# arthurmensch/modl

Hardware: AMD Instinct MI355X
Metric: samples/sec through DictFact.partial_fit at k=256, p=10k (higher is better)
Workload: dtype f32

## Files before the change

### include/modl_hip.h

```cpp
#ifndef MODL_HIP_H
#define MODL_HIP_H

#include <stddef.h>
#include <stdint.h>

#ifdef __cplusplus
extern "C" {
#endif

#define MODL_ABI_VERSION 5

#define MODL_MAX_COMPONENTS 4096

#define MODL_OK 0
#define MODL_EINVAL (-1)
#define MODL_ENOMEM (-2)
#define MODL_ESTATE (-3)
#define MODL_ENOGPU (-4)
#define MODL_ENORCCL (-5)
#define MODL_ERCCL (-6)
#define MODL_ETIMEOUT (-7)

#define MODL_F32 0
#define MODL_F64 1

#define MODL_AGG_MASKED 0
#define MODL_AGG_FULL 1
#define MODL_AGG_AVERAGE 2

#define MODL_OPT_VARIATIONAL 0
#define MODL_OPT_SGD 1

#define MODL_FLAG_NO_RIDER 1
#define MODL_FLAG_GEMM_STAMPS 2

int modl_abi_version(void);
int modl_max_components(void);
int modl_device_count(void);
const char *modl_error_string(int code);
#define MODL_DEBUG_CD_SPARSE_PCT 1
#define MODL_DEBUG_CD_SPLIT 2
#define MODL_DEBUG_CD_STAMPS 3
#define MODL_DEBUG_BCD_ACC 5
#define MODL_DEBUG_ATOM_STAMPS 6
#define MODL_DEBUG_BCD_TINY 7
#define MODL_DEBUG_STAGE_AHEAD 8
#define MODL_DEBUG_BCD_PERSIST 9
#define MODL_DEBUG_STATS_RESIDENT 10
#define MODL_DEBUG_RECSYS_FUSED 11
#define MODL_DEBUG_ATOM_MWG 12
#define MODL_DEBUG_BCD_FEW 13
#define MODL_DEBUG_ATOM_PIPE 14
int modl_debug_set(int what, int64_t value);
int modl_is_diag_build(void);

typedef struct modl_rk modl_rk;
int modl_rk_create(uint64_t seed, modl_rk **out);
void modl_rk_destroy(modl_rk *rk);
int modl_rk_seed(modl_rk *rk, uint64_t seed);
int modl_rk_random(modl_rk *rk, uint32_t *out);
int modl_rk_randint(modl_rk *rk, uint64_t high, int64_t *out);
int modl_rk_double(modl_rk *rk, double *out);
int modl_rk_binomial(modl_rk *rk, int64_t n, double p, int64_t *out);
int modl_rk_permutation(modl_rk *rk, int64_t n, int64_t *h_out);
int modl_rk_get_mt_state(const modl_rk *rk, uint32_t *h_key624, int32_t *pos);
int modl_rk_set_mt_state(modl_rk *rk, const uint32_t *h_key624, int32_t pos);
int modl_rk_shuffle_i64(modl_rk *rk, int64_t *h_x, int64_t n);
int modl_rk_shuffle_trace(modl_rk *rk, int64_t n, int64_t *h_trace, int64_t *h_swaps);
int modl_apply_swaps_rows(void *h_base, int64_t n, size_t row_bytes, const int64_t *h_swaps);
int modl_apply_swaps_rows_device(void *d_base, int64_t n, size_t row_bytes, const int64_t *h_swaps,
                                 void *stream);

typedef struct modl_sampler modl_sampler;
int modl_sampler_create(int64_t range, int rand_size, int replacement, uint64_t seed, modl_sampler **out);
void modl_sampler_destroy(modl_sampler *s);
int modl_sampler_yield_subset(modl_sampler *s, double reduction, int64_t *h_out, int64_t *n_out);
int modl_sampler_get(modl_sampler *s, int64_t *range, int64_t *lim_inf, int64_t *lim_sup, int64_t *h_box);
size_t modl_sampler_state_bytes(const modl_sampler *s);
int modl_sampler_get_state(const modl_sampler *s, void *h_buf, size_t bytes);
int modl_sampler_set_state(modl_sampler *s, const void *h_buf, size_t bytes);

int modl_batch_weight(int64_t count, int64_t batch_size, double learning_rate, double offset, double *out);


size_t modl_enet_regression_workspace(int dtype, int64_t b, int64_t k, int multi_gram);
int modl_enet_regression_single_gram_f32(const float *d_G, float *d_Dx, const float *d_X, int64_t ldx,
                                         int64_t p, float *d_code, const int64_t *d_indices, int64_t b,
                                         int64_t k, float l1_ratio, float alpha, int positive, float tol,
                                         int max_iter, int32_t *d_sweeps, void *d_ws, size_t ws_bytes,
                                         void *stream);
int modl_enet_regression_single_gram_f64(const double *d_G, double *d_Dx, const double *d_X, int64_t ldx,
                                         int64_t p, double *d_code, const int64_t *d_indices, int64_t b,
                                         int64_t k, double l1_ratio, double alpha, int positive, double tol,
                                         int max_iter, int32_t *d_sweeps, void *d_ws, size_t ws_bytes,
                                         void *stream);
int modl_enet_regression_multi_gram_f32(const float *d_G, float *d_Dx, const float *d_X, int64_t ldx,
                                        int64_t p, float *d_code, const int64_t *d_indices, int64_t b,
                                        int64_t k, float l1_ratio, float alpha, int positive, float tol,
                                        int max_iter, int32_t *d_sweeps, void *d_ws, size_t ws_bytes,
                                        void *stream);
int modl_enet_regression_multi_gram_f64(const double *d_G, double *d_Dx, const double *d_X, int64_t ldx,
                                        int64_t p, double *d_code, const int64_t *d_indices, int64_t b,
                                        int64_t k, double l1_ratio, double alpha, int positive, double tol,
                                        int max_iter, int32_t *d_sweeps, void *d_ws, size_t ws_bytes,
                                        void *stream);
int modl_update_G_average_f32(float *d_G_average, const float *d_G, const float *d_w_sample, int64_t b,
                              int64_t k, void *stream);
int modl_update_G_average_f64(double *d_G_average, const double *d_G, const double *d_w_sample, int64_t b,
                              int64_t k, void *stream);

int modl_enet_norm_f32(const float *d_v, int64_t rows, int64_t n, int64_t ld, int64_t inc, float l1_ratio,
                       float *d_out_norm, void *stream);
int modl_enet_norm_f64(const double *d_v, int64_t rows, int64_t n, int64_t ld, int64_t inc, double l1_ratio,
                       double *d_out_norm, void *stream);
int modl_enet_projection_f32(const float *d_v, float *d_out, int64_t rows, int64_t n, int64_t ld, int64_t inc,
                             const float *d_radius, float l1_ratio, void *stream);
int modl_enet_projection_f64(const double *d_v, double *d_out, int64_t rows, int64_t n, int64_t ld,
// ... 202 lines not shown
```

### modl_amd/_lib.py

```python
import ctypes as C
import os

_HERE = os.path.dirname(os.path.abspath(__file__))
LIB_PATH = os.path.join(_HERE, 'libmodl_hip.so')

MODL_F32, MODL_F64 = 0, 1
FLAG_NO_RIDER, FLAG_GEMM_STAMPS = 1, 2
DEBUG_CD_SPARSE_PCT = 1
DEBUG_CD_SPLIT = 2
DEBUG_BCD_ACC = 5
DEBUG_ATOM_STAMPS = 6
DEBUG_BCD_TINY = 7
DEBUG_STAGE_AHEAD = 8
DEBUG_BCD_PERSIST = 9
DEBUG_STATS_RESIDENT = 10
DEBUG_RECSYS_FUSED = 11
DEBUG_ATOM_MWG = 12
DEBUG_BCD_FEW = 13
DEBUG_ATOM_PIPE = 14
AGG = {'masked': 0, 'full': 1, 'average': 2}
OPT = {'variational': 0, 'sgd': 1}


class ModlError(RuntimeError):
    pass


class SomfDesc(C.Structure):
    _fields_ = [('dtype', C.c_int32), ('k', C.c_int32), ('p', C.c_int64), ('n_samples', C.c_int64),
                ('G_agg', C.c_int32), ('Dx_agg', C.c_int32), ('optimizer', C.c_int32), ('code_pos', C.c_int32),
                ('comp_pos', C.c_int32), ('max_iter', C.c_int32), ('code_alpha', C.c_double),
                ('code_l1_ratio', C.c_double), ('comp_l1_ratio', C.c_double), ('tol', C.c_double),
                ('step_size', C.c_double), ('max_batch', C.c_int32), ('flags', C.c_int32)]


class SomfState(C.Structure):
    _fields_ = [('d_Dt', C.c_void_p), ('d_Bt', C.c_void_p), ('d_C', C.c_void_p), ('d_code', C.c_void_p),
                ('d_comp_norm', C.c_void_p), ('d_G', C.c_void_p), ('d_Dx_average', C.c_void_p),
                ('d_G_average', C.c_void_p)]


class SomfBatch(C.Structure):
    _fields_ = [('d_X', C.c_void_p), ('ldx', C.c_int64), ('b', C.c_int32), ('s', C.c_int32),
                ('h_sample_idx', C.c_void_p), ('h_subset', C.c_void_p), ('h_order', C.c_void_p),
                ('h_w_sample', C.c_void_p), ('w', C.c_double), ('reduction', C.c_double),
                ('b_global', C.c_int64)]


class ProfEntry(C.Structure):
    _fields_ = [('name', C.c_char_p), ('ms_total', C.c_double), ('launches', C.c_int64), ('calls', C.c_int64)]


def _load():
    if os.environ.get('MODL_AMD_DIAG') == '1':
        path = os.path.join(_HERE, 'libmodl_hip_diag.so')
        if not os.path.exists(path):
            raise ImportError('modl_amd: MODL_AMD_DIAG=1 but %s is missing (make -C modl_amd/csrc)' % path)
        return C.CDLL(path)
    override = os.environ.get('MODL_HIP_LIBRARY')
    if override:
        if not os.path.exists(override):
            raise ImportError('modl_amd: MODL_HIP_LIBRARY=%s does not exist' % override)
        return C.CDLL(os.path.abspath(override))
    if not os.path.exists(LIB_PATH):
        raise ImportError(
            'modl_amd: %s is missing. Build it with `python -c "import __graft_entry__ as g; g.build()"` '
            'or `make -C modl_amd/csrc` (needs hipcc, --offload-arch=gfx950). There is no CPU fallback.' % LIB_PATH)
    try:
        return C.CDLL(LIB_PATH)
    except OSError as e:
        raise ImportError('modl_amd: cannot load %s: %s' % (LIB_PATH, e))


_vp, _i32, _i64, _u64, _f64, _sz = C.c_void_p, C.c_int32, C.c_int64, C.c_uint64, C.c_double, C.c_size_t
_P = C.POINTER


def bind(lib):
    def _sig(name, restype, *argtypes):
        f = getattr(lib, name)
        f.restype = restype
        f.argtypes = list(argtypes)
        return f

    _sig('modl_abi_version', C.c_int)
    _sig('modl_max_components', C.c_int)
    _sig('modl_device_count', C.c_int)
    _sig('modl_error_string', C.c_char_p, C.c_int)
    _sig('modl_debug_set', C.c_int, C.c_int, _i64)
    _sig('modl_is_diag_build', C.c_int)
# ... 121 lines not shown
```

### modl_amd/csrc/somf_step.hip

```cpp
#include <algorithm>
#include <atomic>
#include <chrono>
#include <condition_variable>
#include <mutex>
#include <thread>
#include <cstdlib>
#include <cstring>
#include <dlfcn.h>
#include <sched.h>
#include <new>
#include <vector>

#include "gemm_dense.hpp"
#include "gemm_wide.hpp"
#include "gemm_resident.hpp"
#include "kernels.hpp"

namespace modl {
std::atomic<int> g_stats_resident{1};

enum Section { SEC_CODE_GEMM = 0, SEC_CODE_SOLVE, SEC_STATS_GEMM, SEC_STATS_APPLY, SEC_DICT, SEC_COUNT };
static const char *kSectionNames[SEC_COUNT] = {"code_gemm", "code_solve", "stats_gemm", "stats_apply", "dict_update"};

constexpr int kStageSlots = 8;
constexpr int kProfPool = 2048;
#ifndef MODL_STAT_BM
#define MODL_STAT_BM 64
#define MODL_STAT_BN 64
#endif
#ifndef MODL_STAT_BK
#define MODL_STAT_BK 0
#endif
constexpr int kStatBM = MODL_STAT_BM, kStatBN = MODL_STAT_BN, kStatBK = MODL_STAT_BK;

template <typename T> struct EpiDxAverage {
    T *Dx; T *avg; const int64_t *idx; const T *w_sample; int64_t k; T alpha;
    __device__ __forceinline__ void operator()(int64_t i, int64_t j, T v) const {
        T *a = avg + (idx ? idx[i] : i) * k + j;
        const T ws = w_sample[i];
        T cur = *a * ((T)1 - ws);
        cur = cur + (alpha * v) * ws;
        *a = cur;
        Dx[i * k + j] = cur;
    }
};

template <typename T> __device__ __forceinline__ bool stats_pow2(T b) {
    if constexpr (sizeof(T) == 4) return (__float_as_uint(b) & 0x007fffffu) == 0 && b > (T)0 && b < (T)1e30;
    else return (__double_as_longlong(b) & 0x000fffffffffffffll) == 0 && b > (T)0 && b < (T)1e300;
}
template <typename T> __device__ __forceinline__ T stats_value(T v, T old, T beta, T wt, T bdiv, int replace, bool p2, T rinv) {
    const T x = replace ? v : wt * v;
    const T q = p2 ? x * rinv : x / bdiv;
    return replace ? q : old * beta + q;
}
template <typename T> struct EpiStats {
    static constexpr bool rmw = true;
    typedef T vec4 __attribute__((ext_vector_type(4)));
    T *out; int64_t ld; T beta, wt, bdiv; int replace; T *mirror;
    __device__ __forceinline__ T load(int64_t m, int64_t n) const { return out[m * ld + n]; }
    __device__ __forceinline__ void store(int64_t m, int64_t n, T v, T old) const {
        const bool p2 = stats_pow2(bdiv);
        const T nv = stats_value(v, old, beta, wt, bdiv, replace, p2, (T)1 / bdiv);
        out[m * ld + n] = nv;
        if (mirror) mirror[m * ld + n] = nv;
    }
    __device__ __forceinline__ void operator()(int64_t m, int64_t n, T v) const { store(m, n, v, load(m, n)); }
    bool vec4_ok() const {
        return ld % 4 == 0 && reinterpret_cast<uintptr_t>(out) % (4 * sizeof(T)) == 0 &&
               reinterpret_cast<uintptr_t>(mirror) % (4 * sizeof(T)) == 0;
    }
    __device__ __forceinline__ vec4 load4(int64_t m, int64_t n) const { return *reinterpret_cast<const vec4 *>(out + m * ld + n); }
    __device__ __forceinline__ void store4(int64_t m, int64_t n, vec4 v, vec4 old) const {
        const bool p2 = stats_pow2(bdiv);
        const T rinv = (T)1 / bdiv;
        vec4 nv;
#pragma unroll
        for (int c = 0; c < 4; ++c) nv[c] = stats_value(v[c], old[c], beta, wt, bdiv, replace, p2, rinv);
        *reinterpret_cast<vec4 *>(out + m * ld + n) = nv;
        if (mirror) *reinterpret_cast<vec4 *>(mirror + m * ld + n) = nv;
    }
};

template <typename T> struct EpiStatsRows {
    static constexpr bool rmw = true;
    T *out; int64_t ld; const int32_t *rows; T beta, wt, bdiv; int replace; T *mirror;
    __device__ __forceinline__ T load(int64_t m, int64_t n) const { return out[(int64_t)rows[m] * ld + n]; }
    __device__ __forceinline__ void store(int64_t m, int64_t n, T v, T old) const {
        const T nv = stats_value(v, old, beta, wt, bdiv, replace, stats_pow2(bdiv), (T)1 / bdiv);
        out[(int64_t)rows[m] * ld + n] = nv;
        if (mirror) mirror[m * ld + n] = nv;
    }
    __device__ __forceinline__ void operator()(int64_t m, int64_t n, T v) const { store(m, n, v, load(m, n)); }
};

template <typename T> struct PrepArgs {
// ... 366 lines not shown
int solve_codes(modl_somf_plan *pl, hipStream_t st, const T *G, int64_t g_stride, const int64_t *g_idx, T *Dx,
                const T *xnorm2, T *code, const int64_t *d_idx, int b, int32_t *d_sweeps, int *nl, T *H0buf, T *Fbuf,
                T *scatter_dst = nullptr, const int64_t *scatter_idx = nullptr, const int64_t *h_gidx = nullptr) {
    const modl_somf_desc &d = pl->d;
    const int k = d.k;
    if (d.code_l1_ratio == 0.0 && chol_blocked(k, sizeof(T), g_stride == 0)) {
        if (g_stride && g_idx && !h_gidx) return MODL_EINVAL;
        T *Linv = reinterpret_cast<T *>(pl->dws + pl->off_Linv);
        MODL_TRY(ridge_solve_wide<T>(st, G, g_stride, h_gidx, Fbuf, Linv, Dx, b, k, (T)d.code_alpha, code, d_idx));
        *nl += 2;
        if (scatter_dst) {
            hipLaunchKernelGGL((scatter_rows_T_kernel<T, int64_t>), dim3((unsigned)b), dim3(256), 0, st, scatter_dst,
                               (int64_t)k, scatter_idx, (int64_t)b, (int64_t)k, Dx, (int64_t)k);
            MODL_LAUNCH_CHECK();
            ++*nl;
        }
        return MODL_OK;
    }
    if (d.code_l1_ratio == 0.0) {
        const int nmat = g_stride ? b : 1;
        if (ridge_small_applies<T>(k)) {
            MODL_TRY(launch_ridge_small<T>(st, G, g_stride, g_idx, Dx, b, k, (T)d.code_alpha, code, d_idx));
            *nl += 1;
        } else {
            MODL_TRY(launch_cholesky<T>(st, G, g_stride, g_idx, Fbuf, k, (T)d.code_alpha, nmat));
            MODL_TRY(launch_chol_solve<T>(st, Fbuf, g_stride ? (int64_t)k * k : 0, Dx, b, k, code, d_idx));
            *nl += 2;
        }
        if (scatter_dst) {
            hipLaunchKernelGGL((scatter_rows_T_kernel<T, int64_t>), dim3((unsigned)b), dim3(256), 0, st, scatter_dst,
                               (int64_t)k, scatter_idx, (int64_t)b, (int64_t)k, code, (int64_t)k);
            MODL_LAUNCH_CHECK();
            ++*nl;
        }
        return MODL_OK;
    }
    const T *H0 = nullptr;
    (void)H0buf;
    CdArgs<T> a;
    a.G = G; a.g_stride = g_stride; a.g_idx = g_idx; a.Dx = Dx; a.xnorm2 = xnorm2; a.H0 = H0; a.code = code;
    a.idx = d_idx;
    a.code2 = scatter_dst; a.idx2 = scatter_idx;
    a.g_pad_rows = (G == reinterpret_cast<const T *>(pl->dws + pl->off_G)) ? 16 : 0;
    if (!g_stride && pl->ld_gpad && k <= 1024) {
        T *Gp = reinterpret_cast<T *>(pl->dws + pl->off_Gpad);
        MODL_TRY(launch_cd_pad_gram<T>(st, G, k, Gp, pl->ld_gpad));
        ++*nl;
        a.G = Gp; a.ldg = pl->ld_gpad; a.g_pad_rows = 16;
    }
    a.sweeps = d_sweeps; a.b = b; a.k = k;
    a.alpha = (T)((T)d.code_alpha * (T)d.code_l1_ratio);
    a.beta = (T)((double)(T)d.code_alpha * (1.0 - (double)(T)d.code_l1_ratio));
    a.tol = (T)d.tol; a.max_iter = d.max_iter; a.positive = d.code_pos;
    if (k > 1024) {
        a.G = G; a.ldg = 0; a.g_pad_rows = 0;
        if (!g_stride) {
            Operand A, B;
            A.ptr = code; A.si = k; A.sk = 1; A.gi = gather64(d_idx);
            B.ptr = G; B.si = k; B.sk = 1;
            EpiStore<T> epi{H0buf, k, (T)1};
            SplitWs none;
            MODL_TRY((launch_gemm<T, EpiStore<T>>(st, A, B, b, k, k, epi, none, nl, 512, 1)));
            a.H0 = H0buf;
        }
        MODL_TRY(launch_cd_wide<T>(st, a));
        ++*nl;
        return MODL_OK;
    }
    if (g_stride && k >= 32 && (cd_split_enabled() || !cd_one_wave_covers(k)) && !cd_split_applies<T>(a)) {
        if (!pl->Gslots) {
            pl->Gslots_bytes = cd_per_sample_scratch_bytes(sizeof(T), d.max_batch, k);
            MODL_HIP(hipMalloc(&pl->Gslots, pl->Gslots_bytes));
            MODL_HIP(hipMemsetAsync(pl->Gslots, 0, pl->Gslots_bytes, st));
        }
        MODL_TRY(launch_cd_per_sample<T>(st, a, static_cast<T *>(pl->Gslots), pl->Gslots_bytes));
        *nl += 2;
        return MODL_OK;
    }
    MODL_TRY(launch_cd<T>(st, a));
    ++*nl;
    return MODL_OK;
}

constexpr int64_t kResidentMinRows = 4096;

template <typename T, class Epi0, class Epi1>
int stats_pair(hipStream_t st, const DenseOperand &A0, const DenseOperand &B0, int64_t M0, int64_t N0, const Epi0 &e0,
               const DenseOperand &A1, const DenseOperand &B1, int64_t M1, int64_t N1, const Epi1 &e1, int64_t K,
               const SplitWs &sws, int *launches, unsigned long long *dbg = nullptr) {
    if constexpr (std::is_same<T, float>::value) {
        auto P0 = plan_stats<Epi0>(A0, B0, M0, N0, K, e0);
        if (P0.ok && M1 >= kResidentMinRows && N1 <= 256 && K % 4 == 0 && !dbg && g_stats_resident.load(std::memory_order_relaxed)) {
            auto W = plan_wide<16, Epi1>(A1, B1, M1, N1, K, e1);
            if (W.ok) {
                static const int ncu = [] {
                    int dev = 0;
                    hipDeviceProp_t prop;
                    if (hipGetDevice(&dev) == hipSuccess && hipGetDeviceProperties(&prop, dev) == hipSuccess)
                        return prop.multiProcessorCount;
                    return 256;
                }();
                return launch_gemm_stats_resident_pair<16, Epi0, Epi1>(st, P0, W, ncu, launches);
            }
        }
        if (P0.ok && cdiv(M1, 64) >= 1024 && !dbg) {
            auto W = plan_wide<32, Epi1>(A1, B1, M1, N1, K, e1);
            if (W.ok) return launch_gemm_stats_wide_pair<32, Epi0, Epi1, 256, 8, 0, true>(st, P0, W, launches);
        }
        auto P1 = plan_stats<Epi1>(A1, B1, M1, N1, K, e1);
        if (P0.ok && P1.ok) {
            P1.dbg = dbg;
            return launch_gemm_stats_pair<Epi0, Epi1>(st, P0, P1, launches);
        }
    }
    DenseProblem<T, Epi0> P0;
    P0.epi = e0;
    bool ok0 = true;
    if (M0 > 0) {
        P0 = plan_dense<T, Epi0>(A0, B0, M0, N0, K, e0, nullptr, 0);
        ok0 = P0.ok;
    }
    auto P1 = plan_dense<T, Epi1>(A1, B1, M1, N1, K, e1, nullptr, 0, 512, 1, kStatBM, kStatBN);
    if (ok0 && P1.ok)
        return launch_gemm_dense_pair<T, true, true, Epi0, true, true, Epi1, kStatBM, kStatBN, kStatBK>(st, P0, P1, launches);
    if (M0 > 0) MODL_TRY((launch_gemm_dense<T, Epi0>(st, A0, B0, M0, N0, K, e0, sws, launches)));
    return launch_gemm_dense<T, Epi1>(st, A1, B1, M1, N1, K, e1, sws, launches);
}

template <typename T>
int phase1(modl_somf_plan *pl, const modl_somf_state *stt, const modl_somf_batch *bt, T *delta, hipStream_t st,
           bool two_phase) {
    const modl_somf_desc &d = pl->d;
    const int k = d.k, b = bt->b;
    const int64_t p = d.p, s = bt->s;
    if (!stt || !stt->d_Dt || !stt->d_code || (two_phase && !delta)) return MODL_EINVAL;
    if (!stt->d_Bt || !stt->d_C || bt->b_global <= 0) return MODL_EINVAL;
    if (d.G_agg == MODL_AGG_FULL && !stt->d_G) return MODL_EINVAL;
    if (d.G_agg == MODL_AGG_AVERAGE && !stt->d_G_average) return MODL_EINVAL;
    if (d.Dx_agg == MODL_AGG_AVERAGE && !stt->d_Dx_average) return MODL_EINVAL;
    MODL_TRY(stage_batch<T>(pl, bt, st));
    ++pl->prof_step;
    char *P = pl->dws + pl->off_params;
    const int64_t *d_idx = pl->has_idx ? reinterpret_cast<const int64_t *>(P + pl->po_idx) : nullptr;
    const int32_t *d_subset = pl->has_subset ? reinterpret_cast<const int32_t *>(P + pl->po_subset) : nullptr;
    const T *d_wsample = reinterpret_cast<const T *>(P + pl->po_wsample);
    const T *X = static_cast<const T *>(bt->d_X);
    const T *Dt = static_cast<const T *>(stt->d_Dt);
    T *code = static_cast<T *>(stt->d_code);
    T *xnorm = reinterpret_cast<T *>(pl->dws + pl->off_xnorm);
    T *Dx = reinterpret_cast<T *>(pl->dws + pl->off_Dx);
    T *H0 = reinterpret_cast<T *>(pl->dws + pl->off_H0);
    T *Gbuf = reinterpret_cast<T *>(pl->dws + pl->off_G);
    T *Fbuf = reinterpret_cast<T *>(pl->dws + pl->off_F);
    SplitWs sws{pl->dws + pl->off_split, pl->split_bytes};
    int32_t *d_sweeps = reinterpret_cast<int32_t *>(pl->dws + pl->off_sweeps);
    if (pl->hist) d_sweeps = pl->hist + (pl->hist_n++ % pl->hist_cap) * (int64_t)d.max_batch;
    pl->last_sweeps_ptr = d_sweeps;
    pl->last_b = b;
    const T red = (T)bt->reduction;

    T *Dsb = reinterpret_cast<T *>(pl->dws + pl->off_Ds);
    T *Xsb = reinterpret_cast<T *>(pl->dws + pl->off_Xs);
    T *codeb = reinterpret_cast<T *>(pl->dws + pl->off_codeb);
    const int64_t s_pad = (s + 3) / 4 * 4;
    const bool cd_on_compact = d.code_l1_ratio != 0.0 && d.G_agg != MODL_AGG_AVERAGE;
    T *cb = codeb;
    if (!d_idx) cb = code;

    T *ws_split = reinterpret_cast<T *>(sws.ptr);
    const size_t ws_elems = sws.bytes / sizeof(T);
    bool ride = false;
    pl->ride_pending = false;
    pl->head_pending = false;
    {
        ProfScope ps(pl, st, SEC_CODE_GEMM);
        const T *Dsrc = Dt, *Xsrc = X;
        int64_t ldxs = bt->ldx;
        const bool need_sub = d_subset && (d.Dx_agg != MODL_AGG_FULL || d.G_agg != MODL_AGG_FULL);
        PrepArgs<T> pa;
        pa.X = X; pa.ldx = bt->ldx; pa.p = p; pa.b = b; pa.xnorm = xnorm; pa.n_norm = (d.code_l1_ratio != 0.0) ? b : 0;
        pa.Dt = Dt; pa.subset = d_subset; pa.s = s; pa.k = k; pa.Ds = Dsb; pa.n_rows = need_sub ? (int)cdiv(s, kPrepRows) : 0;
        pa.s_pad = s_pad; pa.Xs = Xsb; pa.gx = (int)std::min<int64_t>(cdiv(s_pad, 256), 64);
        pa.n_cols = (need_sub && d.Dx_agg != MODL_AGG_FULL) ? pa.gx * b : 0;
        const size_t row_bytes = sizeof(T) * (size_t)p;
        pa.fuse_cols = (pa.n_cols > 0 && pa.n_norm == b && row_bytes <= 64 * 1024 &&
                        reinterpret_cast<uintptr_t>(X) % 16 == 0 && (bt->ldx * sizeof(T)) % 16 == 0) ? 1 : 0;
        if (pa.fuse_cols) pa.n_cols = 0;
        pa.code = code; pa.idx = d_idx; pa.codeb = codeb; pa.n_code = (cd_on_compact && d_idx) ? (int)cdiv(b, kPrepRows) : 0;
        const bool proper = need_sub && s > 0 && s < p;
        ride = proper && d.Dx_agg != MODL_AGG_FULL && !(d.flags & MODL_FLAG_NO_RIDER) && cdiv(p, 64) < 1024;
        if (ride) pl->step_id = (pl->step_id == 0x7fffffff) ? 1 : pl->step_id + 1;
        pa.stamp = ride ? reinterpret_cast<int32_t *>(pl->dws + pl->off_stamp) : nullptr;
        pa.pos = reinterpret_cast<int32_t *>(pl->dws + pl->off_pos);
        pa.step = pl->step_id;
        if (need_sub) {
            Dsrc = Dsb;
            if (d.Dx_agg != MODL_AGG_FULL) { Xsrc = Xsb; ldxs = s_pad; }
        }
        const int n_prep = pa.n_norm + pa.n_rows + pa.n_cols + pa.n_code;
        if (n_prep > 0) {
            hipLaunchKernelGGL((prep_kernel<T>), dim3((unsigned)n_prep), dim3(256), pa.fuse_cols ? row_bytes : 0, st, pa);
            MODL_LAUNCH_CHECK();
            ++ps.launches;
        }
        DenseOperand A, B;
        int64_t Kdim;
        T scale;
        if (d.Dx_agg == MODL_AGG_FULL) {
            A.ptr = X; A.si = bt->ldx; A.sk = 1;
            B.ptr = Dt; B.si = 1; B.sk = k;
            Kdim = p; scale = 1;
        } else {
            A.ptr = Xsrc; A.si = ldxs; A.sk = 1;
            B.ptr = Dsrc; B.si = 1; B.sk = k;
            Kdim = s; scale = red;
        }
        DenseOperand Dg;
        Dg.ptr = Dsrc; Dg.si = 1; Dg.sk = k;
        const bool want_G = d.G_agg != MODL_AGG_FULL;
        bool paired = false;
        if (want_G && A.si != 1) {
            EpiStore<T> epiG{Gbuf, k, red};
            const size_t half = ws_elems / 2;
            constexpr int kPairTarget = 256;
            auto PG = plan_dense<T, EpiStore<T>>(Dg, Dg, k, k, s, epiG, ws_split + half, ws_elems - half, kPairTarget, 64, 64, 64, true);
            if (d.Dx_agg == MODL_AGG_AVERAGE) {
                EpiDxAverage<T> epi{Dx, static_cast<T *>(stt->d_Dx_average), d_idx, d_wsample, k, scale};
                auto PD = plan_dense<T, EpiDxAverage<T>>(A, B, b, k, Kdim, epi, ws_split, half, kPairTarget);
                if (PD.ok && PG.ok) {
                    MODL_TRY((launch_gemm_dense_pair<T, false, true, EpiDxAverage<T>, true, true, EpiStore<T>>(st, PD, PG,
                                                                                                                &ps.launches)));
                    paired = true;
                }
            } else {
                EpiStore<T> epi{Dx, k, scale};
                auto PD = plan_dense<T, EpiStore<T>>(A, B, b, k, Kdim, epi, ws_split, half, kPairTarget);
                if (PD.ok && PG.ok) {
                    MODL_TRY((launch_gemm_dense_pair<T, false, true, EpiStore<T>, true, true, EpiStore<T>>(st, PD, PG,
                                                                                                            &ps.launches)));
                    paired = true;
                }
            }
        }
        if (!paired) {
            if (d.Dx_agg == MODL_AGG_AVERAGE) {
                EpiDxAverage<T> epi{Dx, static_cast<T *>(stt->d_Dx_average), d_idx, d_wsample, k, scale};
                MODL_TRY((launch_gemm_dense<T, EpiDxAverage<T>>(st, A, B, b, k, Kdim, epi, sws, &ps.launches)));
            } else {
                EpiStore<T> epi{Dx, k, scale};
                MODL_TRY((launch_gemm_dense<T, EpiStore<T>>(st, A, B, b, k, Kdim, epi, sws, &ps.launches)));
            }
            if (want_G) {
                EpiStore<T> epi{Gbuf, k, red};
                MODL_TRY((launch_gemm_dense<T, EpiStore<T>>(st, Dg, Dg, k, k, s, epi, sws, &ps.launches)));
            }
        }
        if (d.G_agg == MODL_AGG_AVERAGE) {
            MODL_TRY(launch_update_G_average<T>(st, static_cast<T *>(stt->d_G_average), d_idx, Gbuf, d_wsample, b, k));
            ++ps.launches;
        }
    }
    {
        ProfScope ps(pl, st, SEC_CODE_SOLVE);
        if (d.G_agg == MODL_AGG_AVERAGE) {
            const T *Gavg = static_cast<const T *>(stt->d_G_average);
            MODL_TRY(solve_codes<T>(pl, st, Gavg, (int64_t)k * k, d_idx, Dx, xnorm, code, d_idx, b, d_sweeps,
                                    &ps.launches, H0, Fbuf, nullptr, nullptr, bt->h_sample_idx));
        } else {
            const T *G = (d.G_agg == MODL_AGG_FULL) ? static_cast<const T *>(stt->d_G) : Gbuf;
            if (cd_on_compact) {
                MODL_TRY(solve_codes<T>(pl, st, G, 0, nullptr, Dx, xnorm, cb, nullptr, b, d_sweeps, &ps.launches, H0, Fbuf,
                                        d_idx ? code : nullptr, d_idx));
            } else {
                MODL_TRY(solve_codes<T>(pl, st, G, 0, nullptr, Dx, xnorm, code, d_idx, b, d_sweeps, &ps.launches, H0, Fbuf));
            }
        }
    }
    {
        ProfScope ps(pl, st, SEC_STATS_GEMM);
        if (!cd_on_compact && d_idx) {
            hipLaunchKernelGGL((gather_rows_T_kernel<T, int64_t>), dim3((unsigned)b), dim3(256), 0, st, code, (int64_t)k,
                               d_idx, (int64_t)b, (int64_t)b, (int64_t)k, codeb, (int64_t)k);
            MODL_LAUNCH_CHECK();
            ++ps.launches;
        }
        DenseOperand Cd;
        Cd.ptr = cb; Cd.si = 1; Cd.sk = k;
        DenseOperand Xo;
        Xo.ptr = X; Xo.si = 1; Xo.sk = bt->ldx;
        DenseOperand Xso;
        Xso.ptr = Xsb; Xso.si = 1; Xso.sk = s_pad;
        const int replace = d.optimizer == MODL_OPT_SGD;
        const T beta = (T)(1.0 - bt->w), wt = (T)bt->w, bdiv = (T)bt->b_global;
        T *Bt = static_cast<T *>(stt->d_Bt);
        T *mC = two_phase ? delta : nullptr, *mB = two_phase ? delta + (size_t)k * k : nullptr;
        EpiStats<T> eC{static_cast<T *>(stt->d_C), k, beta, wt, bdiv, replace, mC};
        if (ride) {
            EpiStatsRows<T> eBs{Bt, k, d_subset, beta, wt, bdiv, replace, mB};
            const bool gstamps = (d.flags & MODL_FLAG_GEMM_STAMPS) != 0;
            MODL_TRY((stats_pair<T>(st, Cd, Cd, k, k, eC, Xso, Cd, s, k, eBs, b, sws, &ps.launches,
                                    gstamps ? reinterpret_cast<unsigned long long *>(pl->dws + pl->off_gstamps) : nullptr)));
            StatsRider &R = pl->rider;
            R.X = X; R.ldx = bt->ldx; R.code = cb; R.b = b; R.p = p; R.Bt = stt->d_Bt;
            R.stamp = reinterpret_cast<const int32_t *>(pl->dws + pl->off_stamp); R.step = pl->step_id;
            R.beta = (double)beta; R.wt = (double)wt; R.bdiv = (double)bdiv; R.replace = replace; R.consumed = 0;
            pl->ride_pending = true;
        } else {
            EpiStats<T> eB{Bt, k, beta, wt, bdiv, replace, d_subset ? nullptr : mB};
            MODL_TRY((stats_pair<T>(st, Cd, Cd, k, k, eC, Xo, Cd, p, k, eB, b, sws, &ps.launches)));
            if (two_phase && d_subset && s > 0) {
                hipLaunchKernelGGL((gather_rows_T_kernel<T, int32_t>), dim3((unsigned)s), dim3(256), 0, st, Bt, (int64_t)k,
                                   d_subset, s, s, (int64_t)k, mB, (int64_t)k);
                MODL_LAUNCH_CHECK();
                ++ps.launches;
            }
        }
        if (two_phase) {
            pl->head_pending = true;
            pl->head_elems = (int64_t)k * k + (d_subset ? s : p) * (int64_t)k;
        }
    }
    return MODL_OK;
// ... 850 lines not shown
```

Baseline: 1.161 million.

## Add register-resident split-K MFMA kernel for paired code/Gram products

Adds a specialized kernel for the paired Dx = X·D and G = DᵀD products in the code step. Each block owns a 32x32 tile, loads its K-slice directly from global memory into registers with no LDS staging, splits K across up to 8 waves, and reduces the partial sums through shared memory. The Gram product computes only upper-triangular tiles and mirrors them. The new path is the default when the eligibility checks pass, and a new flag restores the generic paired dense GEMM. The trade-off is heavier register use and a ceiling on K per split, in return for lower tile overhead and roughly half the Gram work.

```diff
diff --git a/include/modl_hip.h b/include/modl_hip.h
--- a/include/modl_hip.h
+++ b/include/modl_hip.h
@@ -33,6 +33,7 @@
 
 #define MODL_FLAG_NO_RIDER 1
 #define MODL_FLAG_GEMM_STAMPS 2
+#define MODL_FLAG_SPLIT_PRODUCTS 4
 
 int modl_abi_version(void);
 int modl_max_components(void);
diff --git a/modl_amd/_lib.py b/modl_amd/_lib.py
--- a/modl_amd/_lib.py
+++ b/modl_amd/_lib.py
@@ -5,7 +5,7 @@
 LIB_PATH = os.path.join(_HERE, 'libmodl_hip.so')
 
 MODL_F32, MODL_F64 = 0, 1
-FLAG_NO_RIDER, FLAG_GEMM_STAMPS = 1, 2
+FLAG_NO_RIDER, FLAG_GEMM_STAMPS, FLAG_SPLIT_PRODUCTS = 1, 2, 4
 DEBUG_CD_SPARSE_PCT = 1
 DEBUG_CD_SPLIT = 2
 DEBUG_BCD_ACC = 5
diff --git a/modl_amd/csrc/gemm_code.hpp b/modl_amd/csrc/gemm_code.hpp
--- /dev/null
+++ b/modl_amd/csrc/gemm_code.hpp
@@ -0,0 +1,220 @@
+#pragma once
+#include "gemm_dense.hpp"
+
+namespace modl {
+
+constexpr int kCodeTile = 32;
+constexpr int kCodeWaves = 8;
+constexpr int kCodeBK = 32;
+constexpr int kCodeNKT = 5;
+constexpr int kCodeMaxKps = 192;
+
+template <class Epi> struct CodeProblem {
+    DenseOperand A, B;
+    int64_t M = 0, N = 0, K = 0, kps = 0;
+    Epi epi;
+    int tn = 0, tm = 0, splits = 1, sym = 0;
+    __host__ __device__ int tiles() const { return sym ? tm * (tm + 1) / 2 : tn * tm; }
+};
+
+template <class Epi>
+CodeProblem<Epi> code_problem(const DenseProblem<float, Epi> &P, bool sym) {
+    CodeProblem<Epi> C;
+    C.A = P.A; C.B = P.B; C.M = P.M; C.N = P.N; C.K = P.K; C.kps = P.kps; C.epi = P.epi;
+    C.tm = (int)cdiv(P.M, kCodeTile); C.tn = (int)cdiv(P.N, kCodeTile);
+    C.splits = P.splits; C.sym = sym ? 1 : 0;
+    return C;
+}
+
+template <class Epi>
+bool code_eligible(const DenseProblem<float, Epi> &P, bool a_along_k) {
+    if (!P.ok || P.A.unal || P.B.unal) return false;
+    if (a_along_k ? P.A.sk != 1 : P.A.si != 1) return false;
+    if (P.B.si != 1) return false;
+    if (P.splits < 1 || P.splits > kCodeWaves) return false;
+    if (P.kps % kCodeBK != 0 || P.kps > kCodeMaxKps) return false;
+    if ((int64_t)kCodeTile * P.A.si + (kCodeMaxKps + 1) * P.A.sk >= ((int64_t)1 << 30)) return false;
+    if ((int64_t)kCodeTile * P.B.si + (kCodeMaxKps + 1) * P.B.sk >= ((int64_t)1 << 30)) return false;
+    return true;
+}
+
+__device__ __forceinline__ void code_swap32(float &a, float &b) {
+    auto r = __builtin_amdgcn_permlane32_swap(__float_as_uint(a), __float_as_uint(b), false, false);
+    a = __uint_as_float(r[0]);
+    b = __uint_as_float(r[1]);
+}
+
+template <bool FULL, int NKT>
+__device__ __forceinline__ void code_load_rows(float (&f)[NKT * (kCodeBK / 2)], const float *base, unsigned sk, unsigned ic,
+                                               int krem, int nkt, int lane) {
+    const unsigned h = lane >> 5;
+#pragma unroll
+    for (int t = 0; t < NKT; ++t)
+        if (t < nkt) {
+#pragma unroll
+            for (int u = 0; u < kCodeBK / 2; ++u) {
+                const int j = t * (kCodeBK / 2) + u;
+                unsigned kl = 2 * j + h;
+                if (!FULL) kl = ((int)kl < krem) ? kl : (unsigned)(krem - 1);
+                f[j] = *reinterpret_cast<const float *>(reinterpret_cast<const char *>(base) + (ic + kl * sk) * 4u);
+            }
+        }
+}
+template <int NKT>
+__device__ __forceinline__ void code_fix_rows(float (&f)[NKT * (kCodeBK / 2)], int krem, int nkt, int lane) {
+    const int h = lane >> 5;
+#pragma unroll
+    for (int t = 0; t < NKT; ++t)
+        if (t < nkt) {
+#pragma unroll
+            for (int u = 0; u < kCodeBK / 2; ++u) {
+                const int j = t * (kCodeBK / 2) + u;
+                f[j] = (2 * j + h < krem) ? f[j] : 0.f;
+            }
+        }
+}
+
+template <bool FULL, int NKT>
+__device__ __forceinline__ void code_load_k(float (&f)[NKT * (kCodeBK / 2)], const float *base, unsigned row, int krem,
+                                            int nkt, int lane) {
+    const unsigned h = lane >> 5;
+#pragma unroll
+    for (int t = 0; t < NKT; ++t)
+        if (t < nkt) {
+#pragma unroll
+            for (int q = 0; q < 4; ++q) {
+                unsigned kl = kCodeBK * t + 8 * q + 4 * h;
+                if (!FULL) kl = ((int)kl < krem) ? kl : 0u;
+                const float4 v = *reinterpret_cast<const float4 *>(reinterpret_cast<const char *>(base) + (row + kl) * 4u);
+                float *d = &f[t * (kCodeBK / 2) + 4 * q];
+                d[0] = v.x; d[1] = v.y; d[2] = v.z; d[3] = v.w;
+            }
+        }
+}
+template <bool FULL, int NKT>
+__device__ __forceinline__ void code_fix_k(float (&f)[NKT * (kCodeBK / 2)], int krem, int nkt, int lane) {
+    const int h = lane >> 5;
+#pragma unroll
+    for (int t = 0; t < NKT; ++t)
+        if (t < nkt) {
+#pragma unroll
+            for (int q = 0; q < 4; ++q) {
+                float *d = &f[t * (kCodeBK / 2) + 4 * q];
+                if (!FULL) {
+                    const int kl = kCodeBK * t + 8 * q + 4 * h;
+#pragma unroll
+                    for (int c = 0; c < 4; ++c) d[c] = (kl + c < krem) ? d[c] : 0.f;
+                }
+                code_swap32(d[0], d[1]);
+                code_swap32(d[2], d[3]);
+                const float x = d[1];
+                d[1] = d[2];
+                d[2] = x;
+            }
+        }
+}
+
+template <class Epi, bool AK, int NKT>
+__device__ __forceinline__ void gemm_code_pass(const CodeProblem<Epi> &P, int64_t m0, int64_t n0, int64_t k_begin, int64_t k_end,
+                                               int lane, Mma<float>::acc_t &acc, Mma<float>::acc_t &acc2) {
+    using MT = Mma<float>;
+    const int krem = (int)(k_end - k_begin), nkt = (krem + kCodeBK - 1) / kCodeBK;
+    const int i = lane & 31;
+    const unsigned ia = (unsigned)((m0 + i < P.M) ? i : P.M - 1 - m0), ib = (unsigned)((n0 + i < P.N) ? i : P.N - 1 - n0);
+    const float *pa = static_cast<const float *>(P.A.ptr) + m0 * P.A.si + k_begin * P.A.sk;
+    const float *pb = static_cast<const float *>(P.B.ptr) + n0 + k_begin * P.B.sk;
+    const unsigned ska = (unsigned)P.A.sk, skb = (unsigned)P.B.sk, rowa = ia * (unsigned)P.A.si;
+    float a[NKT * (kCodeBK / 2)], b[NKT * (kCodeBK / 2)];
+    if (krem == nkt * kCodeBK) {
+        if (AK) code_load_k<true, NKT>(a, pa, rowa, krem, nkt, lane);
+        else code_load_rows<true, NKT>(a, pa, ska, ia, krem, nkt, lane);
+        code_load_rows<true, NKT>(b, pb, skb, ib, krem, nkt, lane);
+        if (AK) code_fix_k<true, NKT>(a, krem, nkt, lane);
+    } else {
+        if (AK) code_load_k<false, NKT>(a, pa, rowa, krem, nkt, lane);
+        else code_load_rows<false, NKT>(a, pa, ska, ia, krem, nkt, lane);
+        code_load_rows<false, NKT>(b, pb, skb, ib, krem, nkt, lane);
+        if (AK) code_fix_k<false, NKT>(a, krem, nkt, lane);
+        else code_fix_rows<NKT>(a, krem, nkt, lane);
+        code_fix_rows<NKT>(b, krem, nkt, lane);
+    }
+#pragma unroll
+    for (int t = 0; t < NKT; ++t)
+        if (t < nkt) {
+#pragma unroll
+            for (int u = 0; u < kCodeBK / 2; ++u) {
+                const int j = t * (kCodeBK / 2) + u;
+                if (u & 1) acc2 = MT::mma(a[j], b[j], acc2);
+                else acc = MT::mma(a[j], b[j], acc);
+            }
+        }
+}
+
+template <class Epi, bool AK>
+__device__ __forceinline__ void gemm_code_tile(const CodeProblem<Epi> &P, int bx, int by, float (*part)[16][64]) {
+    using MT = Mma<float>;
+    const int lane = threadIdx.x & 63, w = __builtin_amdgcn_readfirstlane((int)(threadIdx.x >> 6));
+    const int64_t m0 = (int64_t)by * kCodeTile, n0 = (int64_t)bx * kCodeTile;
+    if (w < P.splits) {
+        const int64_t k_begin = (int64_t)w * P.kps, k_end = (k_begin + P.kps < P.K) ? k_begin + P.kps : P.K;
+        MT::acc_t acc, acc2;
+#pragma unroll
+        for (int r = 0; r < MT::NACC; ++r) { acc[r] = 0; acc2[r] = 0; }
+        constexpr int64_t kPass = kCodeNKT * kCodeBK;
+        gemm_code_pass<Epi, AK, kCodeNKT>(P, m0, n0, k_begin, k_begin + kPass < k_end ? k_begin + kPass : k_end, lane, acc, acc2);
+        if (k_begin + kPass < k_end)
+            gemm_code_pass<Epi, AK, (kCodeMaxKps - kCodeNKT * kCodeBK) / kCodeBK>(P, m0, n0, k_begin + kPass, k_end, lane, acc, acc2);
+#pragma unroll
+        for (int r = 0; r < MT::NACC; ++r) part[w][r][lane] = acc[r] + acc2[r];
+    }
+    __syncthreads();
+    const bool mirror = P.sym && bx > by;
+    const int splits = P.splits;
+    for (int e = (int)threadIdx.x; e < MT::NACC * 64; e += (int)blockDim.x) {
+        const int r = e >> 6, l = e & 63;
+        float x[kCodeWaves];
+#pragma unroll
+        for (int z = 0; z < kCodeWaves; ++z) x[z] = part[z < splits ? z : splits - 1][r][l];
+        float v = x[0];
+        if (splits > 1) {
+            v = 0.f;
+#pragma unroll
+            for (int z = 0; z < kCodeWaves; ++z) v += (z < splits) ? x[z] : 0.f;
+        }
+        const int64_t m = m0 + MT::acc_row(l, r), n = n0 + MT::acc_col(l, r);
+        if (m < P.M && n < P.N) {
+            P.epi(m, n, v);
+            if (mirror) P.epi(n, m, v);
+        }
+    }
+}
+
+template <class Epi0, class Epi1>
+__global__ __launch_bounds__(kCodeWaves * 64) void gemm_code_pair_kernel(CodeProblem<Epi0> P0, CodeProblem<Epi1> P1) {
+    __shared__ float part[kCodeWaves][16][64];
+    int id = (int)blockIdx.x;
+    const int t0 = P0.tiles();
+    if (id < t0) {
+        gemm_code_tile<Epi0, true>(P0, id % P0.tn, id / P0.tn, part);
+    } else {
+        id -= t0;
+        int r = 0;
+        while (id >= P1.tn - r) { id -= P1.tn - r; ++r; }
+        gemm_code_tile<Epi1, false>(P1, r + id, r, part);
+    }
+}
+
+template <class Epi0, class Epi1>
+int launch_gemm_code_pair(hipStream_t stream, const DenseProblem<float, Epi0> &P0, const DenseProblem<float, Epi1> &P1,
+                          int *launches = nullptr) {
+    const CodeProblem<Epi0> C0 = code_problem(P0, false);
+    const CodeProblem<Epi1> C1 = code_problem(P1, true);
+    const int waves = C0.splits > C1.splits ? C0.splits : C1.splits;
+    hipLaunchKernelGGL((gemm_code_pair_kernel<Epi0, Epi1>), dim3((unsigned)(C0.tiles() + C1.tiles())), dim3(64 * waves), 0,
+                       stream, C0, C1);
+    MODL_LAUNCH_CHECK();
+    if (launches) ++*launches;
+    return MODL_OK;
+}
+
+}
diff --git a/modl_amd/csrc/somf_step.hip b/modl_amd/csrc/somf_step.hip
--- a/modl_amd/csrc/somf_step.hip
+++ b/modl_amd/csrc/somf_step.hip
@@ -12,6 +12,7 @@
 #include <vector>
 
 #include "gemm_dense.hpp"
+#include "gemm_code.hpp"
 #include "gemm_wide.hpp"
 #include "gemm_resident.hpp"
 #include "kernels.hpp"
@@ -544,6 +545,19 @@
     return MODL_OK;
 }
 
+template <typename T, class Epi0, class Epi1>
+bool code_route(int32_t flags, const DenseProblem<T, Epi0> &PD, const DenseProblem<T, Epi1> &PG) {
+    if constexpr (std::is_same<T, float>::value)
+        return !(flags & MODL_FLAG_SPLIT_PRODUCTS) && code_eligible(PD, true) && code_eligible(PG, false);
+    else
+        return false;
+}
+template <typename T, class Epi0, class Epi1>
+int launch_code_pair(hipStream_t st, const DenseProblem<T, Epi0> &PD, const DenseProblem<T, Epi1> &PG, int *launches) {
+    if constexpr (std::is_same<T, float>::value) return launch_gemm_code_pair<Epi0, Epi1>(st, PD, PG, launches);
+    else return MODL_EINVAL;
+}
+
 constexpr int64_t kResidentMinRows = 4096;
 
 template <typename T, class Epi0, class Epi1>
@@ -690,16 +704,20 @@
                 EpiDxAverage<T> epi{Dx, static_cast<T *>(stt->d_Dx_average), d_idx, d_wsample, k, scale};
                 auto PD = plan_dense<T, EpiDxAverage<T>>(A, B, b, k, Kdim, epi, ws_split, half, kPairTarget);
                 if (PD.ok && PG.ok) {
-                    MODL_TRY((launch_gemm_dense_pair<T, false, true, EpiDxAverage<T>, true, true, EpiStore<T>>(st, PD, PG,
-                                                                                                                &ps.launches)));
+                    if (code_route<T>(d.flags, PD, PG)) MODL_TRY(launch_code_pair(st, PD, PG, &ps.launches));
+                    else
+                        MODL_TRY((launch_gemm_dense_pair<T, false, true, EpiDxAverage<T>, true, true, EpiStore<T>>(st, PD, PG,
+                                                                                                                    &ps.launches)));
                     paired = true;
                 }
             } else {
                 EpiStore<T> epi{Dx, k, scale};
                 auto PD = plan_dense<T, EpiStore<T>>(A, B, b, k, Kdim, epi, ws_split, half, kPairTarget);
                 if (PD.ok && PG.ok) {
-                    MODL_TRY((launch_gemm_dense_pair<T, false, true, EpiStore<T>, true, true, EpiStore<T>>(st, PD, PG,
-                                                                                                            &ps.launches)));
+                    if (code_route<T>(d.flags, PD, PG)) MODL_TRY(launch_code_pair(st, PD, PG, &ps.launches));
+                    else
+                        MODL_TRY((launch_gemm_dense_pair<T, false, true, EpiStore<T>, true, true, EpiStore<T>>(st, PD, PG,
+                                                                                                                &ps.launches)));
                     paired = true;
                 }
             }
```

Result: faster. 1.176 million, median of 6 (+1.3%).
